# Cibiv/NextGenMap

Hardware: AMD Instinct MI355X
Metric: mapped reads/sec + SW Gcells/sec, 150bp vs GRCh38, at 1/2/4/8 MI355X (higher is better)
Workload: dtype int32

## Files before the change

### include/ngm_pipeline.h

```cpp
#ifndef NGM_PIPELINE_H
#define NGM_PIPELINE_H

#include <stddef.h>
#include <stdint.h>

#ifdef __cplusplus
extern "C" {
#endif

typedef struct ngm_ref ngm_ref;
typedef struct ngm_mapper ngm_mapper;

typedef struct ngm_ref_params {
	int kmer;
	int kmer_skip;
	int bin_size;
} ngm_ref_params;

const char *ngm_pipeline_last_error(void);

ngm_ref *ngm_ref_create(int device, const ngm_ref_params *p, int n_contigs, const char *const *names,
		const uint8_t *const *seqs, const uint64_t *lens);
ngm_ref *ngm_ref_create_from_fasta(int device, const ngm_ref_params *p, const char *path);
ngm_ref *ngm_ref_create_from_cache(int device, const ngm_ref_params *params, const char *fasta_path);
// ... 222 lines not shown
int ngm_debug_select_top1(int device, int n_reads, const uint32_t *base, const uint32_t *count, uint64_t n_cand, const float *scores, const uint32_t *loc,
		const uint32_t *strand_votes, uint32_t *winner, int32_t *mapq, int32_t *n_best, float *best_score);

int ngm_debug_align_finish(void *engine , int mode, int n, const char *const *ref, const char *const *qry, void *out ,
		uint64_t *n_fallback);

int ngm_debug_expand_pairs(int device, int n_reads, const uint32_t *base, const uint32_t *count, uint64_t n_cand, uint32_t *out);

int ngm_debug_pair_select(int device, int n_pairs, const uint32_t *base, const uint32_t *count, uint64_t n_cand, const float *scores, const uint32_t *loc,
		const uint16_t *read_len, int min_insert, int max_insert, float cutoff, int32_t *info, int32_t *mapq, int32_t *n_best, uint32_t counts[4], void *entries, void *tops);

int ngm_mapper_heavy_counters(ngm_mapper *m, uint64_t out[4]);

int ngm_mapper_search_turn_counters(ngm_mapper *m, uint64_t out[3]);

int ngm_mapper_cs_counters(ngm_mapper *m, uint64_t out[3]);

typedef struct ngm_stats_comm ngm_stats_comm;
int ngm_stats_unique_id(char hex[257]);
ngm_stats_comm *ngm_stats_comm_create(int device, int rank, int world, const char *hex);
int ngm_stats_allreduce(ngm_stats_comm *c, int64_t v[8]);
void ngm_stats_comm_destroy(ngm_stats_comm *c);
int ngm_mapper_last_pair_stats(ngm_mapper *m, uint64_t out[3]);

int ngm_mapper_last_kernel_ms(ngm_mapper *m, float ms[8]);
float ngm_mapper_last_order_replay_ms(ngm_mapper *m);

int ngm_mapper_set_argos(ngm_mapper *m, float min_score);
long long ngm_mapper_map_argos(ngm_mapper *m, int n, const char *reads, const char *names, size_t names_bytes, const ngm_sam_read *meta,
		char *out, size_t out_cap, uint64_t stats[3], float *kernel_ms);
// ... 10 lines not shown
```

### nextgenmap_amd/csrc/mapper.cpp

```cpp
#define NGM_SAM_KERNELS
#include "mapper_internal.h"
#define NGM_COV_BATCH_KERNELS
#include "coverage_device.h"
#include "snp_device.h"
#include "count_device.h"
#include "side_output.h"
#include <rocprim/rocprim.hpp>
#include "align_device.h"
#include "gather_device.h"

using ngm::DevGuard;
using ngm::GpuStage;
using ngm::run_cs;
using ngm::cs_host_arrays;
using ngm::candidate_order;
using ngm::candidate_order_wait;

namespace ngm {
StageLock g_stage_lock[16][2];
std::atomic<long long> g_stage_hold_us[3], g_stage_wait_us[3];
}
using ngm::g_stage_hold_us;
using ngm::g_stage_wait_us;

namespace {

int upload_reads(ngm_mapper *m, int n, const char *reads) {
	const size_t bytes = (size_t) n * m->prm.qry_max_len;
	if (m->d_reads.reserve(bytes)) { ngm::pipeline_set_error("out of device memory (reads)"); return -12; }
	MAP_HIP_TRY(hipMemcpyAsync(m->d_reads.p, reads, bytes, hipMemcpyHostToDevice, m->st));
	return 0;
}

std::atomic<int> g_live_mappers{0};
template <typename F>
// ... 86 lines not shown
	if (p->bs_mapping) {
		if (ref->prm.kmer_skip != 0) { ngm::pipeline_set_error("ngm_mapper_create: bisulfite mapping needs a reference index built with kmer_skip 0 (src/PrefixTable.cpp:199-207)"); return nullptr; }
		if (p->mode != 0) { ngm::pipeline_set_error("ngm_mapper_create: '--bs-mapping' and '--end-to-end' can't be used at the same time"); return nullptr; }
		ep.alt_scoring = ep.alt_cigar = NGM_ALT_BISULFITE; ep.match_bonus_tt = p->match_bonus_tt; ep.match_bonus_tc = p->match_bonus_tc;
	}
	if (p->slam_seq) {
		if (p->bs_mapping) { ngm::pipeline_set_error("ngm_mapper_create: '--bs-mapping' and '--slam-seq' can't be used at the same time!"); return nullptr; }
		if (p->personality != NGM_PERSONALITY_LINEAR) { ngm::pipeline_set_error("ngm_mapper_create: '--slam-seq' needs the default (linear-gap) personality: EndToEndAffine produces no per-base records (Align::ExtendedData)"); return nullptr; }
		ep.alt_cigar = NGM_ALT_SLAMSEQ;
		if (p->slam_seq & 2) { ep.alt_scoring = NGM_ALT_SLAMSEQ; ep.match_bonus_tt = p->match_bonus_tt; ep.match_bonus_tc = p->match_bonus_tc; }
	}
	ngm_hip_ctx *eng = ngm_hip_create(ref->device, &ep);
	if (!eng) { ngm::pipeline_set_error("%s", ngm_hip_last_error(nullptr)); return nullptr; }
	ngm_mapper *m = new ngm_mapper();
	++g_live_mappers;
	m->ref = ref; m->prm = *p; m->eng = eng; m->st = eng->stream;
	{
		int lo = 0, hi = 0;
		(void) hipDeviceGetStreamPriorityRange(&lo, &hi);
		if (hipStreamCreateWithPriority(&m->st_hi, hipStreamNonBlocking, hi) != hipSuccess) m->st_hi = nullptr;
	}
	m->max_kfreq = p->max_kfreq > 0 ? p->max_kfreq : ref->auto_max_kfreq;
	for (auto &e : m->ev) (void) hipEventCreate(&e);
	for (auto &e : m->cev) (void) hipEventCreate(&e);
	for (auto &e : m->oev) (void) hipEventCreate(&e);
	if (const char *e = getenv("NGM_HIP_CS_EAGER_ARRAYS")) m->cs_eager_arrays = atoi(e) != 0;
	if (ngm::cs_configure(m, p) != 0) { ngm_mapper_destroy(m); return nullptr; }
	return m;
}

void ngm_mapper_destroy(ngm_mapper *m) {
	if (!m) return;
	if (--g_live_mappers == 0 && getenv("NGM_HIP_HOST_TIMING"))
		fprintf(stderr, "[ngm-hip] GPU stage lock, ms summed over all mappers: search + score held %.1f (waited %.1f) | align held %.1f (waited %.1f) | SAM text held %.1f (waited %.1f)\n",
				g_stage_hold_us[0] / 1e3, g_stage_wait_us[0] / 1e3, g_stage_hold_us[1] / 1e3, g_stage_wait_us[1] / 1e3, g_stage_hold_us[2] / 1e3, g_stage_wait_us[2] / 1e3);
	DevGuard g(m->ref->device);
	(void) hipStreamSynchronize(m->st);
	ngm_bgzf_destroy(m->bz);
	if (m->st_hi) { (void) hipStreamSynchronize(m->st_hi); (void) hipStreamDestroy(m->st_hi); }
	ngm::cs_release(m);
	ngm::argos_release(m);
	m->d_reads.release(); m->d_scores.release(); m->d_best.release(); m->d_pair_read.release();
	m->d_winner.release(); m->d_a_read.release(); m->d_a_loc.release(); m->d_a_sv.release(); m->d_mapq.release(); m->d_nbest.release();
	m->d_records.release(); m->d_runs.release(); m->d_runs_c.release();
	m->d_pair_info.release(); m->p_pair_info.release(); m->d_sam_contig_start.release();
	m->d_pair_out.release(); m->d_pair_top.release(); m->d_pair_tied_n.release(); m->d_pair_list.release(); m->p_pair_out.release(); m->p_pair_top.release(); m->p_pair_tied_n.release();
	m->d_sam_contig_names.release(); m->d_sam_rg.release(); m->d_sam_names.release(); m->d_sam_text.release(); m->d_sam_contig_off.release(); m->d_sam_len.release(); m->d_sam_off.release();
	m->d_sam_quals.release(); m->d_sam_polya.release(); m->d_sam_meta.release(); m->d_sam_refs.release(); m->d_sam_hits.release(); m->p_sam_hits.release(); m->p_sam_refs.release(); m->p_sam_extra.release();
	for (auto &e : m->ev) if (e) (void) hipEventDestroy(e);
	for (auto &e : m->cev) if (e) (void) hipEventDestroy(e);
// ... 582 lines not shown
		if (simple_on_gpu) {
			const size_t npairs = (size_t) n / 2;
			if (m->d_pair_info.reserve(npairs + 1) || m->p_pair_info.reserve(npairs + 1)) { ngm::pipeline_set_error("out of memory (pair selection)"); return -12; }
			if (choice_on_gpu) {
				if (m->d_pair_out.reserve(2 * npairs + 2) || m->d_pair_top.reserve(npairs + 1) || m->d_pair_tied_n.reserve(4) || m->p_pair_tied_n.reserve(4) || m->d_pair_list.reserve(3 * npairs + 2)) {
					ngm::pipeline_set_error("out of memory (pair selection)"); return -12; }
			}
			if (int rc = launch_pair_select(m->st, npairs, m->d_cand_base.p, m->d_cand_count.p, m->d_scores.p, m->d_out_loc.p, m->d_read_len.p, m->prm.min_insert_size, m->prm.max_insert_size,
					m->prm.pair_score_cutoff, m->d_mapq.p, m->d_nbest.p, m->d_pair_info.p, choice_on_gpu, m->d_pair_tied_n.p, m->d_pair_list.p, m->d_pair_out.p, m->d_pair_top.p)) return rc;
			if (choice_on_gpu) {
				MAP_HIP_TRY(hipMemcpyAsync(m->p_pair_tied_n.p, m->d_pair_tied_n.p, 16, hipMemcpyDeviceToHost, m->st));
			}
			MAP_HIP_TRY(hipMemcpyAsync(m->p_pair_info.p, m->d_pair_info.p, (size_t) (n / 2) * 4, hipMemcpyDeviceToHost, m->st));
		}
		MAP_HIP_TRY(hipEventRecord(m->ev[4], m->st));
		MAP_HIP_TRY(hipMemcpyAsync(h_winner, m->d_winner.p, (size_t) n * 4, hipMemcpyDeviceToHost, m->st));
		MAP_HIP_TRY(hipMemcpyAsync(h_mapq, m->d_mapq.p, (size_t) n * 4, hipMemcpyDeviceToHost, m->st));
		MAP_HIP_TRY(hipMemcpyAsync(h_nbest, m->d_nbest.p, (size_t) n * 4, hipMemcpyDeviceToHost, m->st));
		MAP_HIP_TRY(hipMemcpyAsync(h_best, m->d_best.p, (size_t) n * 4, hipMemcpyDeviceToHost, m->st));
		MAP_HIP_TRY(hipMemcpyAsync(h_loc, m->d_out_loc.p, np * 4, hipMemcpyDeviceToHost, m->st));
		MAP_HIP_TRY(hipMemcpyAsync(h_sv, m->d_out_sv.p, np * 4, hipMemcpyDeviceToHost, m->st));
		if (paired) MAP_HIP_TRY(hipMemcpyAsync(h_scores, m->d_scores.p, np * 4, hipMemcpyDeviceToHost, m->st));
		if (int rc = ngm::cs_enqueue_host_arrays(m)) return rc;
		stage_cs.done_after(m->ev[4]);
		MAP_HIP_TRY(hipStreamSynchronize(m->st));
		if (int rc = cs_host_arrays(m)) return rc;
		if (choice_on_gpu) {
			const size_t npairs = (size_t) n / 2;
			const size_t n_small = std::min<size_t>(m->p_pair_tied_n.p[1], npairs), n_large = std::min<size_t>(m->p_pair_tied_n.p[2], npairs), nt = std::min<size_t>(m->p_pair_tied_n.p[0], npairs);
			if (m->p_pair_out.reserve(2 * npairs + 2) || m->p_pair_top.reserve(nt + 1)) { ngm::pipeline_set_error("out of pinned host memory"); return -12; }
			if (n_small) MAP_HIP_TRY(hipMemcpyAsync(m->p_pair_out.p, m->d_pair_out.p, n_small * sizeof(ngm::PairOut), hipMemcpyDeviceToHost, m->st));
			if (n_large) MAP_HIP_TRY(hipMemcpyAsync(m->p_pair_out.p + npairs, m->d_pair_out.p + npairs, n_large * sizeof(ngm::PairOut), hipMemcpyDeviceToHost, m->st));
			if (nt) MAP_HIP_TRY(hipMemcpyAsync(m->p_pair_top.p, m->d_pair_top.p, nt * sizeof(ngm::PairTop), hipMemcpyDeviceToHost, m->st));
			MAP_HIP_TRY(hipStreamSynchronize(m->st));
		}
		lap(1);
		if ((!paired || m->fast_pairing) && m->prm.topn <= 1) {
			std::vector<uint32_t> tied;
			for (int i = 0; i < n; ++i) if (h_nbest[i] != 1 && m->h_count[i] > 1) tied.push_back((uint32_t) i);
// ... 353 lines not shown
		MAP_HIP_TRY(hipEventRecord(m->ev[5], m->st));
		ngm::WindowGeom Ga{r->n_bases - 1, align_buf_len, c >> 1};
		hipLaunchKernelGGL(ngm::gather_pairs_kernel, dim3((na + ngm::kSlots - 1) / ngm::kSlots), dim3(256), 0, m->st, m->d_reads.p, m->d_read_len.p, q,
				r->d_genome, Ga, m->d_a_read.p, m->d_a_loc.p, m->d_a_sv.p, na, eng->RW, eng->FW, eng->packed.p, eng->lens.p, eng->blk_rows.p, alt_dir);
		MAP_HIP_TRY(hipGetLastError());
		MAP_HIP_TRY(hipEventRecord(m->ev[6], m->st));
		const bool was_prof = eng->profiling;
		unsigned long long n_runs_total = 0, n_str_total = 0;
		if (finish) {
			unsigned long long ctr[2] = {0, 0};
			const ngm::AlignFinish fin{m->d_cigout.p, m->d_str.p, scap, m->d_total.p + 8};
			eng->profiling = true;
			if (int rc = ngm::engine_align_packed(eng, mode, na, m->d_records.p, m->d_runs.p, rs, m->st, &fin)) { eng->profiling = was_prof; ngm::pipeline_set_error("%s", ngm_hip_last_error(eng)); return rc; }
			eng->profiling = was_prof;
			MAP_HIP_TRY(hipEventRecord(m->ev[7], m->st));
			MAP_HIP_TRY(hipEventRecord(m->ev[8], m->st));
			MAP_HIP_TRY(hipMemcpyAsync(m->p_cigout.p, m->d_cigout.p, (size_t) na * sizeof(ngm::CigarDevOut), hipMemcpyDeviceToHost, m->st));
			MAP_HIP_TRY(hipMemcpyAsync(ctr, m->d_total.p + 8, 16, hipMemcpyDeviceToHost, m->st));
			stage_align.done_after(m->ev[8]);
			MAP_HIP_TRY(hipStreamSynchronize(m->st));
			n_str_total = std::min<unsigned long long>(ctr[0], scap);
			str_base = n_str_total;
			if (m->p_str.reserve(n_str_total + 1)) { ngm::pipeline_set_error("out of pinned host memory"); return -12; }
			if (n_str_total && !sam) MAP_HIP_TRY(hipMemcpy(m->p_str.p, m->d_str.p, n_str_total, hipMemcpyDeviceToHost));
			if (ctr[1]) {
				if (m->d_runs_c.reserve((size_t) na * rs)) { ngm::pipeline_set_error("out of device memory (runs)"); return -12; }
				MAP_HIP_TRY(hipMemsetAsync(m->d_total.p, 0, 8, m->st));
				if (int rc = ngm::engine_affine_traceback_packed(eng, na, m->d_records.p, m->d_runs.p, rs, m->st)) { ngm::pipeline_set_error("%s", ngm_hip_last_error(eng)); return rc; }
				hipLaunchKernelGGL(ngm::compact_runs_kernel, dim3((na + 255) / 256), dim3(256), 0, m->st, na, m->d_records.p, m->d_runs.p, rs,
						m->d_runs_c.p, m->d_total.p);
				MAP_HIP_TRY(hipGetLastError());
				MAP_HIP_TRY(hipMemcpyAsync(h_rec, m->d_records.p, (size_t) na * 8 * 4, hipMemcpyDeviceToHost, m->st));
				MAP_HIP_TRY(hipMemcpyAsync(&n_runs_total, m->d_total.p, 8, hipMemcpyDeviceToHost, m->st));
				MAP_HIP_TRY(hipStreamSynchronize(m->st));
				if (m->p_runs.reserve(n_runs_total + 1)) { ngm::pipeline_set_error("out of pinned host memory"); return -12; }
				h_runs = m->p_runs.p;
				MAP_HIP_TRY(hipMemcpy(h_runs, m->d_runs_c.p, n_runs_total * 2, hipMemcpyDeviceToHost));
			}
		} else {
		eng->profiling = true;
		if (int rc = ngm::engine_align_packed(eng, mode, na, m->d_records.p, m->d_runs.p, rs, m->st)) { eng->profiling = was_prof; ngm::pipeline_set_error("%s", ngm_hip_last_error(eng)); return rc; }
		eng->profiling = was_prof;
		MAP_HIP_TRY(hipEventRecord(m->ev[7], m->st));
		if (m->d_runs_c.reserve((size_t) na * rs)) { ngm::pipeline_set_error("out of device memory (runs)"); return -12; }
		MAP_HIP_TRY(hipMemsetAsync(m->d_total.p, 0, 8, m->st));
		hipLaunchKernelGGL(ngm::compact_runs_kernel, dim3((na + 255) / 256), dim3(256), 0, m->st, na, m->d_records.p, m->d_runs.p, rs,
				m->d_runs_c.p, m->d_total.p);
		MAP_HIP_TRY(hipGetLastError());
		if (!dev_strings) { MAP_HIP_TRY(hipEventRecord(m->ev[8], m->st)); }
		if (dev_strings) {
			MAP_HIP_TRY(hipMemsetAsync(m->d_total.p + 8, 0, 8, m->st));
			if (affine) hipLaunchKernelGGL(ngm::cigar_strings_kernel<true>, dim3((na + 255) / 256), dim3(256), 0, m->st, na, m->d_records.p, m->d_runs_c.p, eng->packed.p, eng->RW, eng->FW,
					m->d_read_len.p, m->d_a_read.p, m->prm.variant == NGM_VARIANT_OCL_CPU ? 1 : 0, m->prm.hard_clip, m->prm.silent_clip, m->d_cigout.p, m->d_str.p, scap,
					(unsigned long long *) (m->d_total.p + 8), 0);
			else hipLaunchKernelGGL(ngm::cigar_strings_kernel<false>, dim3((na + 255) / 256), dim3(256), 0, m->st, na, m->d_records.p, m->d_runs_c.p, eng->packed.p, eng->RW, eng->FW,
					m->d_read_len.p, m->d_a_read.p, m->prm.variant == NGM_VARIANT_OCL_CPU ? 1 : 0, m->prm.hard_clip, m->prm.silent_clip, m->d_cigout.p, m->d_str.p, scap,
					(unsigned long long *) (m->d_total.p + 8), alt_cigar);
			MAP_HIP_TRY(hipGetLastError());
			MAP_HIP_TRY(hipEventRecord(m->ev[8], m->st));
			MAP_HIP_TRY(hipMemcpyAsync(m->p_cigout.p, m->d_cigout.p, (size_t) na * sizeof(ngm::CigarDevOut), hipMemcpyDeviceToHost, m->st));
			MAP_HIP_TRY(hipMemcpyAsync(&n_str_total, m->d_total.p + 8, 8, hipMemcpyDeviceToHost, m->st));
		}
		MAP_HIP_TRY(hipMemcpyAsync(h_rec, m->d_records.p, (size_t) na * 8 * 4, hipMemcpyDeviceToHost, m->st));
		MAP_HIP_TRY(hipMemcpyAsync(&n_runs_total, m->d_total.p, 8, hipMemcpyDeviceToHost, m->st));
		stage_align.done_after(m->ev[8]);
		MAP_HIP_TRY(hipStreamSynchronize(m->st));
		if (m->p_runs.reserve(n_runs_total + 1)) { ngm::pipeline_set_error("out of pinned host memory"); return -12; }
		h_runs = m->p_runs.p;
		MAP_HIP_TRY(hipMemcpy(h_runs, m->d_runs_c.p, n_runs_total * 2, hipMemcpyDeviceToHost));
		if (dev_strings) {
			n_str_total = std::min<unsigned long long>(n_str_total, scap);
			str_base = n_str_total;
			if (m->p_str.reserve(n_str_total + 1)) { ngm::pipeline_set_error("out of pinned host memory"); return -12; }
			if (n_str_total && !sam) MAP_HIP_TRY(hipMemcpy(m->p_str.p, m->d_str.p, n_str_total, hipMemcpyDeviceToHost));
		}
		}
	}
	stage_align.done();

	lap(3);
// ... 132 lines not shown
			MAP_HIP_TRY(hipMemcpyAsync(&total64, m->d_total.p + 19, 8, hipMemcpyDeviceToHost, m->st));
			MAP_HIP_TRY(hipStreamSynchronize(m->st));
			if (total64 != (unsigned long long) total32) {
				ngm::pipeline_set_error("ngm_mapper_map_sam: the text of this batch of %d reads is %llu bytes, beyond the 32-bit offsets of a batch: use smaller batches", n, total64);
				return -75;
			}
			total = total32;
			if (m->d_sam_text.reserve((size_t) total + 16)) { ngm::pipeline_set_error("out of device memory (SAM text)"); return -12; }
			S.out = m->d_sam_text.p;
			stage_sam.acquire();
			if (bam_slam) hipLaunchKernelGGL(ngm::sam_write_kernel<true>, dim3((units + 255) / 256), dim3(256), 0, m->st, S, units);
			else hipLaunchKernelGGL(ngm::sam_write_kernel<false>, dim3((units + 255) / 256), dim3(256), 0, m->st, S, units);
			MAP_HIP_TRY(hipGetLastError());
		}
		MAP_HIP_TRY(hipEventRecord(e1, m->st));
		ngm::side::Base *const cov_b = ngm::side::base(m->coverage), *const snp_b = ngm::side::base(m->snp), *const count_b = ngm::side::base(m->count);
		auto here = [&](const ngm::side::Base *b) { return b && units > 0 && ngm::side::device(b) == r->device; };
		auto add_here = [&](ngm::side::Base *b, hipEvent_t *ev, auto launch) -> int {
			if (!here(b)) return 0;
			MAP_HIP_TRY(hipEventRecord(ev[0], m->st));
			launch();
			MAP_HIP_TRY(hipGetLastError());
			MAP_HIP_TRY(hipEventRecord(ev[1], m->st));
			return 0;
		};
		auto note_here = [&](ngm::side::Base *b, hipEvent_t *ev) { float t = 0; if (here(b) && hipEventElapsedTime(&t, ev[0], ev[1]) == hipSuccess) ngm::side::note_add_ms(b, t); };
		ngm::cov::Target cov_to{};
		if (here(cov_b)) if (int rc = ngm::coverage_target(m->coverage, &cov_to)) return rc;
		if (int rc = add_here(cov_b, m->cev + 2, [&] {
			hipLaunchKernelGGL(ngm::cov::cov_add_kernel<ngm::cov::CovBatch>, dim3((units + 255) / 256), dim3(256), 0, m->st, ngm::cov::CovBatch{S, units, cov_to.off}, cov_to.counters, cov_to.off, cov_to.n_ref, cov_to.n_aln);
// ... 8 lines not shown
		if (here(count_b)) if (int rc = ngm::count_target(m->count, &count_tab, &count_to)) return rc;
		if (int rc = add_here(count_b, m->cev + 6, [&] {
			hipLaunchKernelGGL(ngm::cnt::count_add_kernel<ngm::cnt::CountBatch>, dim3((units + 255) / 256), dim3(256), 0, m->st, ngm::cnt::CountBatch{ngm::snp::SnpBatch{S, units}}, count_tab, count_to);
		})) return rc;
		const bool cov_away = cov_b && units > 0 && !here(cov_b), snp_away = snp_b && units > 0 && !here(snp_b), count_away = count_b && units > 0 && !here(count_b);
		if (cov_away || snp_away || count_away) {
			if (m->d_cov_mask.reserve((size_t) units)) { ngm::pipeline_set_error("out of device memory (coverage)"); return -12; }
			hipLaunchKernelGGL(ngm::cov::cov_mask_kernel, dim3((units + 255) / 256), dim3(256), 0, m->st, S, units, m->d_cov_mask.p);
			MAP_HIP_TRY(hipGetLastError());
		}
		unsigned long long ctr[7] = {0, 0, 0, 0, 0, 0, 0};
		MAP_HIP_TRY(hipMemcpyAsync(ctr, m->d_total.p + 16, 56, hipMemcpyDeviceToHost, m->st));
		m->sam_text_bytes = total;
		const bool bam = m->sam_opt.bam != 0;
		if (!bam && total <= sam->out_cap && total > 0) MAP_HIP_TRY(hipMemcpyAsync(sam->out, m->d_sam_text.p, (size_t) total, hipMemcpyDeviceToHost, m->st));
		stage_sam.done_after(e1);
		MAP_HIP_TRY(hipStreamSynchronize(m->st));
		sam->text_bytes = (long long) total;
		note_here(cov_b, m->cev + 2); note_here(snp_b, m->cev + 4); note_here(count_b, m->cev + 6);
		if (cov_away || snp_away || count_away)
			if (int rc = side_outputs_away(m, cov_away, snp_away, count_away, n, q, units, paired, hits, sam_refs, (size_t) str_base + extra.size(), sam)) return rc;
		float bgzf_ms = 0.f;
		if (bam && total > 0) {
			if (m->sorter) {
				int rc;
				if (ngm::bam_sort_device(m->sorter) == r->device) rc = ngm::bam_sort_add_device(m->sorter, m->batch_seq, m->d_sam_text.p, (size_t) total, m->d_sam_off.p, (size_t) units);
				else {
					m->sorter_host.resize((size_t) total);
					MAP_HIP_TRY(hipMemcpy(m->sorter_host.data(), m->d_sam_text.p, (size_t) total, hipMemcpyDeviceToHost));
					rc = ngm_bam_sort_add(m->sorter, m->batch_seq, m->sorter_host.data(), (size_t) total);
				}
// ... 283 lines not shown
```

### nextgenmap_amd/csrc/mapper_argos.cpp

```cpp
#include "mapper_internal.h"
#include <rocprim/rocprim.hpp>
#include "argos_device.h"

using ngm::DevGuard;
using ngm::GpuStage;

namespace ngm {
void argos_release(ngm_mapper *m) {
	m->d_argos_starts.release(); m->d_argos_loff.release(); m->d_argos_gkeys.release(); m->d_argos_ord.release(); m->d_argos_nsurv.release();
	m->d_argos_npos.release(); m->d_argos_list.release(); m->d_argos_llist.release(); m->d_argos_gvals.release(); m->d_argos_hord.release();
	m->d_argos_hoff.release(); m->d_argos_cls.release(); m->d_argos_ctr.release(); m->p_argos_cls.release(); m->p_argos_nsurv.release();
	for (auto &e : m->aev) if (e) { (void) hipEventDestroy(e); e = nullptr; }
}
}

namespace {
inline uint64_t pow2_at_least(uint32_t v) { uint64_t p = 1; while (p < v) p <<= 1; return p; }

bool argos_sort_like_reference(std::vector<uint32_t> &v, const float *score, const uint32_t *rank) {
	struct Rec { float s; uint32_t i; };
	thread_local std::vector<Rec> recs;
	bool known = rank != nullptr;
	for (uint32_t c : v) known = known && rank[c] != ngm::kArgosRankUnknown;
	if (known) std::sort(v.begin(), v.end(), [&](uint32_t x, uint32_t y) { return rank[x] < rank[y]; });
// ... 77 lines not shown

	const uint32_t cap = (uint32_t) std::max<long>(1, std::min<long>(ngm::kArgosLdsCap, ngm::test_limit("argos_lds_cap", ngm::kArgosLdsCap)));
	const uint32_t lds_keys = (uint32_t) pow2_at_least(cap);
	ngm::ArgosArgs A{};
	A.n = n; A.list = nullptr; A.cand_base = m->d_cand_base.p; A.cand_count = m->d_cand_count.p; A.scores = m->d_scores.p; A.read_len = m->d_read_len.p;
	A.rank = nullptr; A.min_opt = m->argos_min; A.match = (float) m->prm.match_bonus; A.lds_cap = cap; A.lds_keys = lds_keys;
	A.ord = m->d_argos_ord.p; A.n_surv = m->d_argos_nsurv.p; A.n_pos = m->d_argos_npos.p; A.cls = m->d_argos_cls.p; A.counters = m->d_argos_ctr.p;
	MAP_HIP_TRY(hipMemsetAsync(m->d_argos_ctr.p, 0, 4 * sizeof(unsigned long long), m->st));
	MAP_HIP_TRY(hipEventRecord(m->aev[0], m->st));
	hipLaunchKernelGGL(ngm::argos_order_kernel<false>, dim3((unsigned) n), dim3(ngm::kArgosThreadsLds), (size_t) lds_keys * 12, m->st, A);
	MAP_HIP_TRY(hipGetLastError());
	std::vector<uint32_t> longs;
	for (int i = 0; i < n; ++i) if (m->h_count[i] > cap) longs.push_back((uint32_t) i);
	if (int rc = argos_long_launch(m, A, longs)) return rc;
	MAP_HIP_TRY(hipEventRecord(m->aev[1], m->st));
	MAP_HIP_TRY(hipMemcpyAsync(m->p_argos_cls.p, m->d_argos_cls.p, (size_t) n, hipMemcpyDeviceToHost, m->st));
	MAP_HIP_TRY(hipMemcpyAsync(m->p_argos_nsurv.p, m->d_argos_nsurv.p, (size_t) n * 4, hipMemcpyDeviceToHost, m->st));
	stage.done_after(m->aev[1]);
	MAP_HIP_TRY(hipStreamSynchronize(m->st));

	uint64_t cls_n[3] = {0, 0, 0};
	std::vector<uint32_t> need, s_lds, s_long, h_list;
	for (int i = 0; i < n; ++i) {
		if (m->p_argos_nsurv.p[i] == 0) continue;
		const uint8_t c = m->p_argos_cls.p[i];
		++cls_n[c];
		if (c == ngm::kArgosU) continue;
		need.push_back((uint32_t) i);
		if (c == ngm::kArgosH) h_list.push_back((uint32_t) i);
		else if (m->h_count[i] > cap) s_long.push_back((uint32_t) i);
		else s_lds.push_back((uint32_t) i);
	}
	GpuStage stage_txt(m, 1, false, 2);
// ... 64 lines not shown
	MAP_HIP_TRY(hipMemcpyAsync(&total32, m->d_sam_off.p + n, 4, hipMemcpyDeviceToHost, m->st));
	MAP_HIP_TRY(hipMemcpyAsync(ctr, m->d_argos_ctr.p, sizeof(ctr), hipMemcpyDeviceToHost, m->st));
	MAP_HIP_TRY(hipStreamSynchronize(m->st));
	if (ctr[3] != (unsigned long long) total32) {
		ngm::pipeline_set_error("ngm_mapper_map_argos: the text of this batch of %d reads is %llu bytes, beyond the 32-bit offsets of a batch: use smaller batches", n, ctr[3]);
		return -75;
	}
	const uint64_t total = total32;
	if (total > 0) {
		if (m->d_sam_text.reserve((size_t) total + 16)) { ngm::pipeline_set_error("out of device memory (argos text)"); return -12; }
		T.out = m->d_sam_text.p;
		hipLaunchKernelGGL(ngm::argos_write_kernel, dim3((n + 255) / 256), dim3(256), 0, m->st, T);
		MAP_HIP_TRY(hipGetLastError());
	}
	MAP_HIP_TRY(hipEventRecord(m->aev[3], m->st));
	m->sam_text_bytes = total;
	if (total > 0 && total <= out_cap && out) MAP_HIP_TRY(hipMemcpyAsync(out, m->d_sam_text.p, (size_t) total, hipMemcpyDeviceToHost, m->st));
	stage_txt.done_after(m->aev[3]);
	MAP_HIP_TRY(hipStreamSynchronize(m->st));
	m->argos_unknown += ctr[0];
	for (int c = 0; c < 3; ++c) m->argos_ctr[c] += cls_n[c];
	m->argos_ctr[3] += ctr[2];
	if (stats) { stats[0] = (uint64_t) n; stats[1] = ctr[1]; stats[2] = 0; }
	auto et = [](hipEvent_t a, hipEvent_t b) { float t = 0; return hipEventElapsedTime(&t, a, b) == hipSuccess ? t : 0.f; };
	if (kernel_ms) *kernel_ms = et(m->aev[0], m->aev[1]) + et(m->aev[2], m->aev[3]);
	m->ms[0] = m->cs_kernel_ms;
	m->ms[7] = et(m->ev[0], m->ev[1]);
	if (np > 0) { m->ms[1] = et(m->ev[1], m->ev[2]); m->ms[2] = et(m->ev[2], m->ev[3]); }
	return (long long) total;
}

int ngm_argos_prolog(const ngm_ref *ref, uint64_t total_reads, char *out, size_t cap) {
	if (!ref) return -22;
// ... 46 lines not shown
```

### nextgenmap_amd/csrc/mapper_internal.h

```cpp
#pragma once

#include <algorithm>
#include <atomic>
#include <chrono>
#include <climits>
#include <cmath>
#include <cstdlib>
#include <cstdio>
#include <cstring>
#include <condition_variable>
#include <mutex>
#include <numeric>
#include <thread>
#include <vector>

#include <string.h>
#include <ctype.h>
#include <sched.h>
#include "../../include/ngm_pipeline.h"
#include "refindex.h"
#include "engine_internal.h"
#include "cigar_md.h"
#include "cigar_device.h"
#include "cs_device.h"
// ... 136 lines not shown
		ngm::PinnedBuf<T> b;
		T &operator[](size_t i) { return b.p[i]; }
		const T &operator[](size_t i) const { return b.p[i]; }
		T *data() { return b.p; }
	};
	HostArr<uint32_t> h_base, h_count;
	HostArr<float> h_maxv;
	uint64_t n_cand = 0;
	bool cs_eager_arrays = false;
	int cs_arrays_state = 0;
	int canon_per_cu = 0;
	const void *canon_fn = nullptr;
	size_t canon_lds = 0;
	uint64_t np_seen_max = 0;
	uint64_t turn_dbg[3] = {0, 0, 0};
	hipEvent_t ev[10] = {};
	float ms[8] = {};
};

namespace ngm {

struct DevGuard {
	int prev = -1;
	explicit DevGuard(int d) { if (hipGetDevice(&prev) != hipSuccess) prev = -1; if (prev != d) (void) hipSetDevice(d); else prev = -1; }
	~DevGuard() { if (prev >= 0) (void) hipSetDevice(prev); }
};

struct StageLock { std::mutex mu; };
extern StageLock g_stage_lock[16][2];
extern std::atomic<long long> g_stage_hold_us[3], g_stage_wait_us[3];
struct GpuStage {
	ngm_mapper *m;
	int kind, slot;
	bool held = false;
	StageLock *ch = nullptr;
	std::chrono::steady_clock::time_point t_acq;
	static int mode() { static const int v = getenv("NGM_HIP_GPU_STAGE_LOCK") ? atoi(getenv("NGM_HIP_GPU_STAGE_LOCK")) : 1; return v; }
	GpuStage(ngm_mapper *m_, int kind_ = 0, bool now = true, int slot_ = -1) : m(m_), kind(kind_), slot(slot_ < 0 ? kind_ : slot_) {
		ch = &g_stage_lock[(unsigned) m->ref->device & 15u][mode() == 2 ? kind : 0];
		if (now) acquire();
	}
	~GpuStage() { release(); }
	void acquire() {
		if (mode() == 0 || held) return;
		const auto t0 = std::chrono::steady_clock::now();
		ch->mu.lock();
		held = true;
		t_acq = std::chrono::steady_clock::now();
		g_stage_wait_us[slot] += std::chrono::duration_cast<std::chrono::microseconds>(t_acq - t0).count();
	}
	void release() {
		if (!held) return;
		g_stage_hold_us[slot] += std::chrono::duration_cast<std::chrono::microseconds>(std::chrono::steady_clock::now() - t_acq).count();
		held = false;
		ch->mu.unlock();
	}
	void done_after(hipEvent_t ev) { if (held) (void) hipEventSynchronize(ev); release(); }
	void done() { release(); }
};

int cs_configure(ngm_mapper *m, const ngm_mapper_params *p);
int run_cs(ngm_mapper *m, int n, GpuStage *stage = nullptr, bool defer_host_arrays = false);
int cs_enqueue_host_arrays(ngm_mapper *m);
int cs_host_arrays(ngm_mapper *m);
int candidate_order(ngm_mapper *m, const std::vector<uint32_t> &list, uint64_t np, uint32_t **h_rank, bool wait = true);
int candidate_order_wait(ngm_mapper *m, uint32_t **h_rank);
void cs_release(ngm_mapper *m);
long test_limit(const char *key, long dflt);

int score_candidates(ngm_mapper *m, int n, uint64_t np, int alt_dir);
void argos_release(ngm_mapper *m);

// ... 2 lines not shown
```

### nextgenmap_amd/pipeline.py

```python
import ctypes as C

import numpy as np

from .engine import NgmHipError, load_library


class RefParams(C.Structure):
    _fields_ = [("kmer", C.c_int), ("kmer_skip", C.c_int), ("bin_size", C.c_int)]


class MapperParams(C.Structure):
    _fields_ = [("qry_max_len", C.c_int), ("corridor", C.c_int), ("match_bonus", C.c_int), ("mismatch_penalty", C.c_int),
                ("gap_read_penalty", C.c_int), ("gap_ref_penalty", C.c_int), ("mode", C.c_int), ("variant", C.c_int),
                ("sensitivity", C.c_float), ("kmer_min", C.c_float), ("max_cmrs", C.c_int), ("max_kfreq", C.c_int),
                ("hard_clip", C.c_int), ("silent_clip", C.c_int), ("personality", C.c_int), ("gap_extend_penalty", C.c_int),
                ("min_insert_size", C.c_int), ("max_insert_size", C.c_int), ("pair_score_cutoff", C.c_float),
                ("topn", C.c_int), ("strata", C.c_int), ("bs_mapping", C.c_int), ("bs_cutoff", C.c_int), ("bs_read_skip", C.c_int),
                ("match_bonus_tt", C.c_int), ("match_bonus_tc", C.c_int), ("slam_seq", C.c_int)]


class SamOptions(C.Structure):
    _fields_ = [("paired", C.c_int), ("min_insert_size", C.c_int), ("max_insert_size", C.c_int), ("min_mq", C.c_int),
                ("min_identity", C.c_float), ("min_residues", C.c_float), ("no_unal", C.c_int), ("rg_id", C.c_char_p),
                ("bs_mapping", C.c_int), ("slam_seq", C.c_int), ("bam", C.c_int)]
# ... 59 lines not shown
        lib.ngm_ref_convert.argtypes = [C.c_void_p, C.c_uint64, C.POINTER(C.c_int), C.POINTER(C.c_uint64)]
        lib.ngm_mapper_create.restype = C.c_void_p
        lib.ngm_mapper_create.argtypes = [C.c_void_p, C.POINTER(MapperParams)]
        lib.ngm_mapper_destroy.argtypes = [C.c_void_p]
        lib.ngm_mapper_cs.argtypes = [C.c_void_p, C.c_int, C.c_void_p, C.c_void_p, C.c_void_p]
        lib.ngm_mapper_cs_fetch.argtypes = [C.c_void_p, C.c_void_p, C.c_void_p, C.c_void_p]
        lib.ngm_mapper_map_se.argtypes = [C.c_void_p, C.c_int, C.c_void_p, C.c_void_p, C.c_void_p, C.c_void_p]
        lib.ngm_mapper_map_se_resident.argtypes = [C.c_void_p, C.c_int, C.c_void_p, C.c_void_p, C.c_void_p, C.c_void_p, C.c_void_p]
        lib.ngm_mapper_map_pe_resident.argtypes = [C.c_void_p, C.c_int, C.c_void_p, C.c_void_p, C.c_void_p, C.c_void_p, C.c_void_p]
        lib.ngm_mapper_cs_counters.argtypes = [C.c_void_p, C.c_void_p]
        lib.ngm_mapper_path_counters.argtypes = [C.c_void_p, C.c_void_p]
        lib.ngm_mapper_order_table_reads.argtypes = [C.c_void_p, C.c_void_p]
        lib.ngm_mapper_heavy_counters.argtypes = [C.c_void_p, C.c_void_p]
        lib.ngm_mapper_search_turn_counters.argtypes = [C.c_void_p, C.c_void_p]
        lib.ngm_mapper_last_kernel_ms.argtypes = [C.c_void_p, C.POINTER(C.c_float)]
        lib.ngm_mapper_last_order_replay_ms.restype = C.c_float
        lib.ngm_mapper_last_order_replay_ms.argtypes = [C.c_void_p]
        lib.ngm_mapper_set_argos.argtypes = [C.c_void_p, C.c_float]
        lib.ngm_mapper_map_argos.restype = C.c_longlong
        lib.ngm_mapper_map_argos.argtypes = [C.c_void_p, C.c_int, C.c_void_p, C.c_void_p, C.c_size_t, C.c_void_p, C.c_void_p, C.c_size_t,
                                             C.c_void_p, C.POINTER(C.c_float)]
        lib.ngm_mapper_sam_fetch.argtypes = [C.c_void_p, C.c_void_p, C.c_size_t]
        lib.ngm_mapper_set_sam_options.argtypes = [C.c_void_p, C.c_void_p]
        lib.ngm_mapper_map_sam_trimmed.restype = C.c_longlong
        lib.ngm_mapper_map_sam_trimmed.argtypes = [C.c_void_p, C.c_int, C.c_void_p, C.c_void_p, C.c_void_p, C.c_size_t, C.c_void_p, C.c_void_p,
                                                   C.c_void_p, C.c_size_t, C.c_void_p, C.POINTER(C.c_float)]
        lib.ngm_argos_prolog.argtypes = [C.c_void_p, C.c_uint64, C.c_void_p, C.c_size_t]
        lib.ngm_mapper_argos_counters.argtypes = [C.c_void_p, C.c_void_p]
        lib.ngm_mapper_argos_path_counters.argtypes = [C.c_void_p, C.c_void_p]
        lib.ngm_debug_argos_order.argtypes = [C.c_uint32, C.c_void_p, C.c_void_p, C.c_float, C.c_int, C.c_int, C.c_void_p, C.c_void_p]
# ... 49 lines not shown
        lib.ngm_count_add.argtypes = [C.c_void_p, C.c_void_p, C.c_void_p, C.c_void_p, C.c_char_p, C.c_void_p, C.c_char_p, C.c_char_p, C.c_void_p, C.c_size_t]
        lib.ngm_count_mask.argtypes = [C.c_void_p, C.c_void_p, C.c_void_p, C.c_size_t]
        lib.ngm_count_finish.argtypes = [C.c_void_p]
        lib.ngm_count_read.restype = C.c_longlong
        lib.ngm_count_read.argtypes = [C.c_void_p, C.c_void_p, C.c_size_t]
        lib.ngm_count_stats.argtypes = [C.c_void_p, C.c_void_p, C.c_void_p]
        lib.ngm_mapper_set_count.argtypes = [C.c_void_p, C.c_void_p]
        _bound = True
    return lib


def _err():
    return NgmHipError(_lib().ngm_pipeline_last_error().decode())


class Bgzf:

    def __init__(self, device=0):
        self._h = _lib().ngm_bgzf_create(device)
        if not self._h:
            raise _err()

    def compress(self, data):
        lib = _lib()
        data = bytes(data)
        cap = lib.ngm_bgzf_bound(len(data))
        out = C.create_string_buffer(cap)
        n = lib.ngm_bgzf_compress(self._h, data, len(data), out, cap)
        if n < 0:
            raise _err()
# ... 628 lines not shown
```

Baseline: 60.63 million.

## Hand over GPU stage lock via stream-wait events instead of host event sync

```diff
diff --git a/include/ngm_pipeline.h b/include/ngm_pipeline.h
--- a/include/ngm_pipeline.h
+++ b/include/ngm_pipeline.h
@@ -260,6 +260,17 @@
 
 int ngm_mapper_search_turn_counters(ngm_mapper *m, uint64_t out[3]);
 
+typedef struct ngm_turn_log_entry {
+	uint64_t seq;
+	int32_t channel;
+	int32_t kind;
+	int32_t mapper;
+	int32_t has_end;
+	int32_t has_gap;
+	float begin_ms, end_ms, gap_ms;
+} ngm_turn_log_entry;
+int ngm_debug_turn_log(int device, ngm_turn_log_entry *out, int cap);
+
 int ngm_mapper_cs_counters(ngm_mapper *m, uint64_t out[3]);
 
 typedef struct ngm_stats_comm ngm_stats_comm;
diff --git a/nextgenmap_amd/csrc/mapper.cpp b/nextgenmap_amd/csrc/mapper.cpp
--- a/nextgenmap_amd/csrc/mapper.cpp
+++ b/nextgenmap_amd/csrc/mapper.cpp
@@ -19,6 +19,89 @@
 namespace ngm {
 StageLock g_stage_lock[16][2];
 std::atomic<long long> g_stage_hold_us[3], g_stage_wait_us[3];
+static std::mutex g_turn_origin_mu;
+static hipEvent_t g_turn_origin[16];
+
+void GpuStage::acquire() {
+	if (mode() == 0 || held) return;
+	const auto t0 = std::chrono::steady_clock::now();
+	ch->mu.lock();
+	held = true; marked = false;
+	t_acq = std::chrono::steady_clock::now();
+	g_stage_wait_us[slot] += std::chrono::duration_cast<std::chrono::microseconds>(t_acq - t0).count();
+	turn = &ch->ring[ch->turns % kTurnRing];
+	turn->seq = ch->turns++; turn->mapper = m->id; turn->kind = slot;
+	turn->used = true; turn->has_begin = turn->has_end = false;
+	if (ch->tail && hipStreamWaitEvent(m->st, ch->tail, 0) != hipSuccess) { (void) hipGetLastError(); (void) hipEventSynchronize(ch->tail); }
+	if (!logging()) return;
+	const unsigned dev = (unsigned) m->ref->device & 15u;
+	{
+		std::lock_guard<std::mutex> lk(g_turn_origin_mu);
+		if (!g_turn_origin[dev] && hipEventCreate(&g_turn_origin[dev]) == hipSuccess && hipEventRecord(g_turn_origin[dev], m->st) != hipSuccess) {
+			(void) hipEventDestroy(g_turn_origin[dev]); g_turn_origin[dev] = nullptr;
+		}
+	}
+	if (!turn->begin && hipEventCreate(&turn->begin) != hipSuccess) { turn->begin = nullptr; return; }
+	turn->has_begin = hipEventRecord(turn->begin, m->st) == hipSuccess;
+}
+
+hipError_t GpuStage::mark_end() {
+	if (!held) return hipSuccess;
+	if (!turn->end) { const hipError_t e = hipEventCreate(&turn->end); if (e != hipSuccess) { turn->end = nullptr; return e; } }
+	const hipError_t e = hipEventRecord(turn->end, m->st);
+	marked = turn->has_end = e == hipSuccess;
+	return e;
+}
+
+void GpuStage::release() {
+	if (!held) return;
+	const bool was_marked = marked;
+	if (host_handover()) {
+		if (!was_marked && logging()) (void) mark_end();
+		if (marked) (void) hipEventSynchronize(turn->end);
+		ch->tail = nullptr;
+	} else {
+		if (!marked) (void) mark_end();
+		if (marked) ch->tail = turn->end;
+		else { (void) hipGetLastError(); (void) hipStreamSynchronize(m->st); ch->tail = nullptr; }
+	}
+	g_stage_hold_us[slot] += std::chrono::duration_cast<std::chrono::microseconds>(std::chrono::steady_clock::now() - t_acq).count();
+	held = false; turn = nullptr;
+	ch->mu.unlock();
+}
+}
+
+extern "C" int ngm_debug_turn_log(int device, ngm_turn_log_entry *out, int cap) {
+	if (device < 0 || cap < 0 || (cap > 0 && !out)) return -22;
+	if (!ngm::GpuStage::logging()) return 0;
+	ngm::DevGuard g(device);
+	const unsigned dev = (unsigned) device & 15u;
+	hipEvent_t origin;
+	{ std::lock_guard<std::mutex> lk(ngm::g_turn_origin_mu); origin = ngm::g_turn_origin[dev]; }
+	if (!origin || hipEventQuery(origin) != hipSuccess) { (void) hipGetLastError(); return 0; }
+	int w = 0;
+	for (int c = 0; c < 2; ++c) {
+		ngm::StageLock &ch = ngm::g_stage_lock[dev][c];
+		std::lock_guard<std::mutex> lk(ch.mu);
+		const uint64_t first = ch.turns > (uint64_t) ngm::kTurnRing ? ch.turns - ngm::kTurnRing : 0;
+		const ngm::TurnEntry *prev = nullptr;
+		for (uint64_t s = first; s < ch.turns; ++s) {
+			const ngm::TurnEntry &t = ch.ring[s % ngm::kTurnRing];
+			auto complete = [](hipEvent_t e) { if (hipEventQuery(e) == hipSuccess) return true; (void) hipGetLastError(); return false; };
+			const bool ok = t.used && t.seq == s && t.has_begin && complete(t.begin) && (!t.has_end || complete(t.end));
+			if (ok && w < cap) {
+				ngm_turn_log_entry &o = out[w];
+				o.seq = s; o.channel = c; o.kind = t.kind; o.mapper = t.mapper; o.has_end = t.has_end ? 1 : 0; o.has_gap = 0;
+				o.begin_ms = o.end_ms = o.gap_ms = 0.f;
+				if (hipEventElapsedTime(&o.begin_ms, origin, t.begin) != hipSuccess) { (void) hipGetLastError(); prev = nullptr; continue; }
+				if (t.has_end && hipEventElapsedTime(&o.end_ms, origin, t.end) != hipSuccess) { (void) hipGetLastError(); o.has_end = 0; }
+				if (prev && hipEventElapsedTime(&o.gap_ms, prev->end, t.begin) == hipSuccess) o.has_gap = 1;
+				++w;
+			}
+			prev = (ok && t.has_end) ? &t : nullptr;
+		}
+	}
+	return w;
 }
 using ngm::g_stage_hold_us;
 using ngm::g_stage_wait_us;
@@ -135,6 +218,8 @@
 	if (!eng) { ngm::pipeline_set_error("%s", ngm_hip_last_error(nullptr)); return nullptr; }
 	ngm_mapper *m = new ngm_mapper();
 	++g_live_mappers;
+	static std::atomic<int> next_id{0};
+	m->id = ++next_id;
 	m->ref = ref; m->prm = *p; m->eng = eng; m->st = eng->stream;
 	{
 		int lo = 0, hi = 0;
@@ -153,8 +238,8 @@
 void ngm_mapper_destroy(ngm_mapper *m) {
 	if (!m) return;
 	if (--g_live_mappers == 0 && getenv("NGM_HIP_HOST_TIMING"))
-		fprintf(stderr, "[ngm-hip] GPU stage lock, ms summed over all mappers: search + score held %.1f (waited %.1f) | align held %.1f (waited %.1f) | SAM text held %.1f (waited %.1f)\n",
-				g_stage_hold_us[0] / 1e3, g_stage_wait_us[0] / 1e3, g_stage_hold_us[1] / 1e3, g_stage_wait_us[1] / 1e3, g_stage_hold_us[2] / 1e3, g_stage_wait_us[2] / 1e3);
+		fprintf(stderr, "[ngm-hip] GPU stage lock, HOST ms with the mutex (enqueuing; not the time the kernels ran%s), summed over all mappers: search + score held %.1f (waited %.1f) | align held %.1f (waited %.1f) | SAM text held %.1f (waited %.1f)\n",
+				GpuStage::host_handover() ? " -- NGM_HIP_TURN_HOST_HANDOVER: until the turn's last kernel has ended" : "", g_stage_hold_us[0] / 1e3, g_stage_wait_us[0] / 1e3, g_stage_hold_us[1] / 1e3, g_stage_wait_us[1] / 1e3, g_stage_hold_us[2] / 1e3, g_stage_wait_us[2] / 1e3);
 	DevGuard g(m->ref->device);
 	(void) hipStreamSynchronize(m->st);
 	ngm_bgzf_destroy(m->bz);
@@ -767,6 +852,7 @@
 			MAP_HIP_TRY(hipMemcpyAsync(m->p_pair_info.p, m->d_pair_info.p, (size_t) (n / 2) * 4, hipMemcpyDeviceToHost, m->st));
 		}
 		MAP_HIP_TRY(hipEventRecord(m->ev[4], m->st));
+		MAP_HIP_TRY(stage_cs.mark_end());
 		MAP_HIP_TRY(hipMemcpyAsync(h_winner, m->d_winner.p, (size_t) n * 4, hipMemcpyDeviceToHost, m->st));
 		MAP_HIP_TRY(hipMemcpyAsync(h_mapq, m->d_mapq.p, (size_t) n * 4, hipMemcpyDeviceToHost, m->st));
 		MAP_HIP_TRY(hipMemcpyAsync(h_nbest, m->d_nbest.p, (size_t) n * 4, hipMemcpyDeviceToHost, m->st));
@@ -775,7 +861,7 @@
 		MAP_HIP_TRY(hipMemcpyAsync(h_sv, m->d_out_sv.p, np * 4, hipMemcpyDeviceToHost, m->st));
 		if (paired) MAP_HIP_TRY(hipMemcpyAsync(h_scores, m->d_scores.p, np * 4, hipMemcpyDeviceToHost, m->st));
 		if (int rc = ngm::cs_enqueue_host_arrays(m)) return rc;
-		stage_cs.done_after(m->ev[4]);
+		stage_cs.done();
 		MAP_HIP_TRY(hipStreamSynchronize(m->st));
 		if (int rc = cs_host_arrays(m)) return rc;
 		if (choice_on_gpu) {
@@ -1159,10 +1245,10 @@
 			if (int rc = ngm::engine_align_packed(eng, mode, na, m->d_records.p, m->d_runs.p, rs, m->st, &fin)) { eng->profiling = was_prof; ngm::pipeline_set_error("%s", ngm_hip_last_error(eng)); return rc; }
 			eng->profiling = was_prof;
 			MAP_HIP_TRY(hipEventRecord(m->ev[7], m->st));
-			MAP_HIP_TRY(hipEventRecord(m->ev[8], m->st));
+			MAP_HIP_TRY(stage_align.mark_end());
 			MAP_HIP_TRY(hipMemcpyAsync(m->p_cigout.p, m->d_cigout.p, (size_t) na * sizeof(ngm::CigarDevOut), hipMemcpyDeviceToHost, m->st));
 			MAP_HIP_TRY(hipMemcpyAsync(ctr, m->d_total.p + 8, 16, hipMemcpyDeviceToHost, m->st));
-			stage_align.done_after(m->ev[8]);
+			stage_align.done();
 			MAP_HIP_TRY(hipStreamSynchronize(m->st));
 			n_str_total = std::min<unsigned long long>(ctr[0], scap);
 			str_base = n_str_total;
@@ -1192,7 +1278,7 @@
 		hipLaunchKernelGGL(ngm::compact_runs_kernel, dim3((na + 255) / 256), dim3(256), 0, m->st, na, m->d_records.p, m->d_runs.p, rs,
 				m->d_runs_c.p, m->d_total.p);
 		MAP_HIP_TRY(hipGetLastError());
-		if (!dev_strings) { MAP_HIP_TRY(hipEventRecord(m->ev[8], m->st)); }
+		if (!dev_strings) { MAP_HIP_TRY(stage_align.mark_end()); }
 		if (dev_strings) {
 			MAP_HIP_TRY(hipMemsetAsync(m->d_total.p + 8, 0, 8, m->st));
 			if (affine) hipLaunchKernelGGL(ngm::cigar_strings_kernel<true>, dim3((na + 255) / 256), dim3(256), 0, m->st, na, m->d_records.p, m->d_runs_c.p, eng->packed.p, eng->RW, eng->FW,
@@ -1202,13 +1288,13 @@
 					m->d_read_len.p, m->d_a_read.p, m->prm.variant == NGM_VARIANT_OCL_CPU ? 1 : 0, m->prm.hard_clip, m->prm.silent_clip, m->d_cigout.p, m->d_str.p, scap,
 					(unsigned long long *) (m->d_total.p + 8), alt_cigar);
 			MAP_HIP_TRY(hipGetLastError());
-			MAP_HIP_TRY(hipEventRecord(m->ev[8], m->st));
+			MAP_HIP_TRY(stage_align.mark_end());
 			MAP_HIP_TRY(hipMemcpyAsync(m->p_cigout.p, m->d_cigout.p, (size_t) na * sizeof(ngm::CigarDevOut), hipMemcpyDeviceToHost, m->st));
 			MAP_HIP_TRY(hipMemcpyAsync(&n_str_total, m->d_total.p + 8, 8, hipMemcpyDeviceToHost, m->st));
 		}
 		MAP_HIP_TRY(hipMemcpyAsync(h_rec, m->d_records.p, (size_t) na * 8 * 4, hipMemcpyDeviceToHost, m->st));
 		MAP_HIP_TRY(hipMemcpyAsync(&n_runs_total, m->d_total.p, 8, hipMemcpyDeviceToHost, m->st));
-		stage_align.done_after(m->ev[8]);
+		stage_align.done();
 		MAP_HIP_TRY(hipStreamSynchronize(m->st));
 		if (m->p_runs.reserve(n_runs_total + 1)) { ngm::pipeline_set_error("out of pinned host memory"); return -12; }
 		h_runs = m->p_runs.p;
@@ -1371,6 +1457,7 @@
 			MAP_HIP_TRY(hipGetLastError());
 		}
 		MAP_HIP_TRY(hipEventRecord(e1, m->st));
+		MAP_HIP_TRY(stage_sam.mark_end());
 		ngm::side::Base *const cov_b = ngm::side::base(m->coverage), *const snp_b = ngm::side::base(m->snp), *const count_b = ngm::side::base(m->count);
 		auto here = [&](const ngm::side::Base *b) { return b && units > 0 && ngm::side::device(b) == r->device; };
 		auto add_here = [&](ngm::side::Base *b, hipEvent_t *ev, auto launch) -> int {
@@ -1409,7 +1496,7 @@
 		m->sam_text_bytes = total;
 		const bool bam = m->sam_opt.bam != 0;
 		if (!bam && total <= sam->out_cap && total > 0) MAP_HIP_TRY(hipMemcpyAsync(sam->out, m->d_sam_text.p, (size_t) total, hipMemcpyDeviceToHost, m->st));
-		stage_sam.done_after(e1);
+		stage_sam.done();
 		MAP_HIP_TRY(hipStreamSynchronize(m->st));
 		sam->text_bytes = (long long) total;
 		note_here(cov_b, m->cev + 2); note_here(snp_b, m->cev + 4); note_here(count_b, m->cev + 6);
diff --git a/nextgenmap_amd/csrc/mapper_argos.cpp b/nextgenmap_amd/csrc/mapper_argos.cpp
--- a/nextgenmap_amd/csrc/mapper_argos.cpp
+++ b/nextgenmap_amd/csrc/mapper_argos.cpp
@@ -115,9 +115,10 @@
 	for (int i = 0; i < n; ++i) if (m->h_count[i] > cap) longs.push_back((uint32_t) i);
 	if (int rc = argos_long_launch(m, A, longs)) return rc;
 	MAP_HIP_TRY(hipEventRecord(m->aev[1], m->st));
+	MAP_HIP_TRY(stage.mark_end());
 	MAP_HIP_TRY(hipMemcpyAsync(m->p_argos_cls.p, m->d_argos_cls.p, (size_t) n, hipMemcpyDeviceToHost, m->st));
 	MAP_HIP_TRY(hipMemcpyAsync(m->p_argos_nsurv.p, m->d_argos_nsurv.p, (size_t) n * 4, hipMemcpyDeviceToHost, m->st));
-	stage.done_after(m->aev[1]);
+	stage.done();
 	MAP_HIP_TRY(hipStreamSynchronize(m->st));
 
 	uint64_t cls_n[3] = {0, 0, 0};
@@ -212,9 +213,10 @@
 		MAP_HIP_TRY(hipGetLastError());
 	}
 	MAP_HIP_TRY(hipEventRecord(m->aev[3], m->st));
+	MAP_HIP_TRY(stage_txt.mark_end());
 	m->sam_text_bytes = total;
 	if (total > 0 && total <= out_cap && out) MAP_HIP_TRY(hipMemcpyAsync(out, m->d_sam_text.p, (size_t) total, hipMemcpyDeviceToHost, m->st));
-	stage_txt.done_after(m->aev[3]);
+	stage_txt.done();
 	MAP_HIP_TRY(hipStreamSynchronize(m->st));
 	m->argos_unknown += ctr[0];
 	for (int c = 0; c < 3; ++c) m->argos_ctr[c] += cls_n[c];
diff --git a/nextgenmap_amd/csrc/mapper_internal.h b/nextgenmap_amd/csrc/mapper_internal.h
--- a/nextgenmap_amd/csrc/mapper_internal.h
+++ b/nextgenmap_amd/csrc/mapper_internal.h
@@ -174,6 +174,7 @@
 	size_t canon_lds = 0;
 	uint64_t np_seen_max = 0;
 	uint64_t turn_dbg[3] = {0, 0, 0};
+	int id = 0;
 	hipEvent_t ev[10] = {};
 	float ms[8] = {};
 };
@@ -186,36 +187,41 @@
 	~DevGuard() { if (prev >= 0) (void) hipSetDevice(prev); }
 };
 
-struct StageLock { std::mutex mu; };
+constexpr int kTurnRing = 256;
+struct TurnEntry {
+	hipEvent_t begin = nullptr, end = nullptr;
+	uint64_t seq = 0;
+	int mapper = 0, kind = 0;
+	bool used = false, has_begin = false, has_end = false;
+};
+struct StageLock {
+	std::mutex mu;
+	hipEvent_t tail = nullptr;
+	uint64_t turns = 0;
+	TurnEntry ring[kTurnRing];
+};
 extern StageLock g_stage_lock[16][2];
 extern std::atomic<long long> g_stage_hold_us[3], g_stage_wait_us[3];
 struct GpuStage {
 	ngm_mapper *m;
 	int kind, slot;
-	bool held = false;
+	bool held = false, marked = false;
 	StageLock *ch = nullptr;
+	TurnEntry *turn = nullptr;
 	std::chrono::steady_clock::time_point t_acq;
 	static int mode() { static const int v = getenv("NGM_HIP_GPU_STAGE_LOCK") ? atoi(getenv("NGM_HIP_GPU_STAGE_LOCK")) : 1; return v; }
+	static bool host_handover() { static const bool v = getenv("NGM_HIP_TURN_HOST_HANDOVER") && atoi(getenv("NGM_HIP_TURN_HOST_HANDOVER")) != 0; return v; }
+	static bool logging() { static const bool v = getenv("NGM_HIP_TURN_LOG") && atoi(getenv("NGM_HIP_TURN_LOG")) != 0; return v; }
 	GpuStage(ngm_mapper *m_, int kind_ = 0, bool now = true, int slot_ = -1) : m(m_), kind(kind_), slot(slot_ < 0 ? kind_ : slot_) {
 		ch = &g_stage_lock[(unsigned) m->ref->device & 15u][mode() == 2 ? kind : 0];
 		if (now) acquire();
 	}
 	~GpuStage() { release(); }
-	void acquire() {
-		if (mode() == 0 || held) return;
-		const auto t0 = std::chrono::steady_clock::now();
-		ch->mu.lock();
-		held = true;
-		t_acq = std::chrono::steady_clock::now();
-		g_stage_wait_us[slot] += std::chrono::duration_cast<std::chrono::microseconds>(t_acq - t0).count();
-	}
-	void release() {
-		if (!held) return;
-		g_stage_hold_us[slot] += std::chrono::duration_cast<std::chrono::microseconds>(std::chrono::steady_clock::now() - t_acq).count();
-		held = false;
-		ch->mu.unlock();
-	}
-	void done_after(hipEvent_t ev) { if (held) (void) hipEventSynchronize(ev); release(); }
+	GpuStage(const GpuStage &) = delete;
+	GpuStage &operator=(const GpuStage &) = delete;
+	void acquire();
+	hipError_t mark_end();
+	void release();
 	void done() { release(); }
 };
 
diff --git a/nextgenmap_amd/pipeline.py b/nextgenmap_amd/pipeline.py
--- a/nextgenmap_amd/pipeline.py
+++ b/nextgenmap_amd/pipeline.py
@@ -97,6 +97,7 @@
         lib.ngm_mapper_heavy_counters.argtypes = [C.c_void_p, C.c_void_p]
         lib.ngm_mapper_search_turn_counters.argtypes = [C.c_void_p, C.c_void_p]
         lib.ngm_mapper_last_kernel_ms.argtypes = [C.c_void_p, C.POINTER(C.c_float)]
+        lib.ngm_debug_turn_log.argtypes = [C.c_int, C.c_void_p, C.c_int]
         lib.ngm_mapper_last_order_replay_ms.restype = C.c_float
         lib.ngm_mapper_last_order_replay_ms.argtypes = [C.c_void_p]
         lib.ngm_mapper_set_argos.argtypes = [C.c_void_p, C.c_float]
@@ -176,6 +177,18 @@
     return NgmHipError(_lib().ngm_pipeline_last_error().decode())
 
 
+TURN_DTYPE = np.dtype([("seq", "u8"), ("channel", "i4"), ("kind", "i4"), ("mapper", "i4"), ("has_end", "i4"), ("has_gap", "i4"),
+                       ("begin_ms", "f4"), ("end_ms", "f4"), ("gap_ms", "f4")], align=True)
+
+
+def turn_log(device=0):
+    out = np.zeros(2 * 256, TURN_DTYPE)
+    n = _lib().ngm_debug_turn_log(int(device), out.ctypes.data, out.shape[0])
+    if n < 0:
+        raise _err()
+    return out[:n].copy()
+
+
 class Bgzf:
 
     def __init__(self, device=0):
```

Measured after the change: 60.23 million. No clear change (-0.7%).
